# parseablehq/parseable

Hardware: AMD Instinct MI355X
Metric: rows/sec scanned (SELECT...WHERE...GROUP BY, Parseable parquet dialect) (higher is better)
Workload: dtype int64; 1 GPU; c2s; query=SELECT host,count(*),max(latency) WHERE ts BETWEEN ... GROUP BY host, rows_per_gpu=100000000, parallelism=dp1

## Files before the change

### parseable_amd/csrc/gpuq.cpp

```cpp
#include "../../include/gpuq.h"
#include "catalog.h"
#include "where.h"
#include "meta.h"
#include "kernels_api.h"
#include "dev_types.h"

#include <hip/hip_runtime.h>
#include <fcntl.h>
#include <sys/mman.h>
#include <sys/stat.h>
#include <unistd.h>

#include <algorithm>
#include <array>
#include <atomic>
#include <functional>
#include <cstring>
#include <thread>
#include <map>
#include <memory>
#include <mutex>
#include <string>
#include <unordered_map>
#include <vector>
// ... 301 lines not shown
  gpuq_ctx* ctx = nullptr;
  std::vector<std::unique_ptr<MappedFile>> files;
  std::vector<ColPlan> cols;
  std::vector<PredPlan> preds;
  std::vector<AggPlan> aggs;
  std::vector<int> group_cols;
  std::vector<int> projection;
  bool is_projection = false;
  int ts_col = -1;
  int64_t limit = -1;
  std::vector<Partition> parts;
  int32_t n_groups = 0;
  int32_t n_fsum = 0;
  bool has_hash = false;
  bool needs_cascade = false;
  bool has_numkey = false;
  std::vector<std::string> pinned_keys;
  int64_t m_cache_hit_bytes = 0;
  bool fused_count = false;
  bool fused_valagg = false;
  int valagg_col = -1;
  bool valagg_late = false;
  int valagg_blocks = 1024;
  bool exec_dbg = false;
  std::vector<int> distinct_aggs;
  bool has_tree = false;
  WhereTree where;
  std::vector<int> pred_ctx;
  struct WOr { int node; int ctx; int level; std::vector<int> terms; };
  struct WFold { int node; int ctx; int col; };
  struct WCtx { std::vector<int> ors; };
  std::vector<WCtx> ctxs;
  std::vector<WOr> wors;
  std::vector<WFold> wfolds;
  int n_wbufs = 0;
  int ctx_of(int pidx) const { return has_tree ? pred_ctx[pidx] : 0; }
  uint64_t distinct_bitmap_bits = DISTINCT_BITMAP_BITS;
  uint64_t distinct_lds_bits = DISTINCT_LDS_BITS;
  uint32_t distinct_pair_cap = DISTINCT_PAIR_CAP;
  bool distinct_force_hash = false;
  std::mutex mu;
  int64_t m_rows_scanned = 0, m_rows_out = 0, m_kernel_ns = 0, m_exec_ns = 0,
          m_load_ns = 0, m_decomp_ns = 0, m_hbm_est = 0;
  ~gpuq_plan();
};

// ... 1677 lines not shown
            part.dictv_pool[t.dictv_pool_base + k] =
                rank_of_gid[(size_t)part.dictv_pool[t.dictv_pool_base + k]];
  }

  {
    bool aggs_ok = true;
    for (auto& ap : plan->aggs) aggs_ok &= (ap.kind == AGGK_COUNT_STAR);
    plan->fused_count = plan->group_cols.size() == 1 && aggs_ok &&
                        plan->preds.empty() && plan->n_groups <= 8192 &&
                        !plan->cols[plan->group_cols[0]].is_bin &&
                        !plan->cols[plan->group_cols[0]].hash_mode &&
                        !plan->cols[plan->group_cols[0]].numeric_key;
  }

  for (auto& part : plan->parts) {
    part.col_null_free.assign(plan->cols.size(), 1);
    for (auto& t : part.chunks)
      if (t.cm->null_count != 0) part.col_null_free[t.col_idx] = 0;
  }

  plan->exec_dbg = getenv("GPUQ_PLAN_DEBUG") != nullptr;
  if (const char* e = getenv("GPUQ_VALAGG_BLOCKS"))
    plan->valagg_blocks = std::max(1, atoi(e));
  if (const char* e = getenv("GPUQ_DISTINCT_BITMAP_BITS"))
    plan->distinct_bitmap_bits =
        std::min<uint64_t>(strtoull(e, nullptr, 10), 1ull << 31);
  if (const char* e = getenv("GPUQ_DISTINCT_LDS_BITS"))
    plan->distinct_lds_bits =
        std::min<uint64_t>(strtoull(e, nullptr, 10), 64 * 1024 * 8);
  if (const char* e = getenv("GPUQ_DISTINCT_PAIR_CAP"))
    plan->distinct_pair_cap = (uint32_t)std::min<uint64_t>(
        std::max<uint64_t>(strtoull(e, nullptr, 10), 1), DISTINCT_PAIR_CAP);
  if (const char* e = getenv("GPUQ_DISTINCT_FORCE_HASH"))
    plan->distinct_force_hash = atoi(e) != 0;
  if (!plan->distinct_aggs.empty()) plan->fused_count = false;
  if (!plan->is_projection && !getenv("GPUQ_NO_FUSED_VALAGG") &&
      plan->distinct_aggs.empty() &&
      plan->group_cols.size() == 1 && plan->aggs.size() == 2 &&
      plan->aggs[0].kind == AGGK_COUNT_STAR && plan->n_fsum == 0 &&
      (plan->aggs[1].kind == AGGK_SUM_I64 || plan->aggs[1].kind == AGGK_MIN_I64 ||
       plan->aggs[1].kind == AGGK_MAX_I64) &&
      plan->aggs[1].cnt_is_presence && !plan->needs_cascade) {
    const int vc = plan->aggs[1].col_idx;
    const auto& c = plan->cols[vc];
    const auto& kc = plan->cols[plan->group_cols[0]];
    bool ok = c.phys == PT_INT64 && !c.is_bin && !c.hash_mode &&
// ... 800 lines not shown

  {
    std::lock_guard<std::mutex> g(plan->mu);
    plan->m_kernel_ns += (int64_t)(ms_total * 1e6);
    plan->m_decomp_ns += (int64_t)(ms_decomp * 1e6);
    plan->m_exec_ns += now_ns() - t0;
    plan->m_rows_out += k;
  }
  return 0;
}

}

extern "C" int32_t gpuq_plan_execute(gpuq_plan* plan, int32_t pi,
                                     struct ArrowArrayStream* out) try {
  if (!plan || pi < 0 || pi >= (int32_t)plan->parts.size()) return -1;
  Partition& part = plan->parts[pi];
  if (!part.loaded) {
    if (gpuq_plan_load(plan, pi) != 0) return -1;
  }
  HIP_TRY(hipSetDevice(part.device));
  hipStream_t st = part.stream;
  int64_t t0 = now_ns();

  hipEvent_t ev0, ev1, ev_decomp;
  HIP_TRY(hipEventCreate(&ev0));
  HIP_TRY(hipEventCreate(&ev1));
  HIP_TRY(hipEventCreate(&ev_decomp));

  const bool need_mask = !plan->preds.empty() && !part.pred_ranges.empty();
  HIP_TRY(hipMemsetAsync(part.d_err, 0, 4, st));
  if (need_mask) HIP_TRY(hipMemsetAsync(part.d_mask, 1, part.n_rows, st));
  int64_t n_groups_exec = plan->n_groups;
  bool cascaded = false;
  std::vector<uint32_t> level_claimed;
  std::vector<char> distinct_bitmap(plan->distinct_aggs.size(), 0);
  auto key_card = [&](int ci) -> int64_t {
    const auto& kc = plan->cols[ci];
    return kc.is_bin ? (int64_t)kc.nbins + 1
           : (kc.hash_mode || kc.numeric_key)
               ? (int64_t)part.hash_claimed[ci] + 1
               : (int64_t)kc.gdict.size() + 1;
  };
  if (plan->fused_count)
    launch_init_table(st, part.d_table, plan->n_groups, (int)plan->aggs.size(),
                      part.d_agg_kind);
// ... 7 lines not shown
      part.d_res_lane, (int64_t)part.res_lane.size(),
      part.d_res_wave, (int)part.res_wave.size(),
      part.d_piece_pool, part.d_brs,
      part.d_pagebrs, (int)part.pagebrs.size(), part.d_err});
  HIP_TRY(hipEventRecord(ev_decomp, st));

  if (plan->fused_count) {
    int key_col = plan->group_cols[0];
    auto it = part.tasks.find({TK_DICT_GID, key_col});
    if (it != part.tasks.end())
      launch_dict_count(st, part.d_dec, part.d_pages, part.d_ids[it->first],
                        (int)it->second.size(), part.d_remap, part.d_table,
                        plan->n_groups, (int)plan->aggs.size(), part.d_err);
    HIP_TRY(hipEventRecord(ev1, st));
  } else {
  auto run_task = [&](const std::pair<const std::pair<int, int>,
                                      std::vector<int32_t>>& kv,
                      uint8_t* mk) {
    const int kind = tk_kind(kv.first.first), kctx = tk_ctx_of(kv.first.first);
    const int col = kv.first.second;
    int n = (int)kv.second.size();
    int32_t* ids = part.d_ids[kv.first];
    const uint8_t* d_lut = part.d_lut;
    if (kind == TK_DICT_MASK) {
      const auto& lc = plan->cols[col].lut_ctxs;
      d_lut += (size_t)(std::find(lc.begin(), lc.end(), kctx) - lc.begin()) *
               part.lut_pool.size();
    }
    if (part.col_null_free[col]) {
      switch (kind) {
        case TK_DICT_GID: {
          auto it = part.d_valid.find(col);
          launch_dict_gid(st, part.d_dec, part.d_pages, ids, n, part.d_remap,
                          part.d_gid[col],
                          it != part.d_valid.end() ? it->second : nullptr,
                          nullptr, 2, part.d_err);
          return;
        }
        case TK_DICT_VAL:
          launch_dict_i64(st, part.d_dec, part.d_pages, ids, n, part.d_dictv,
                          part.d_val[col], part.d_valid[col], nullptr, 2,
                          part.d_err);
          return;
        case TK_PLAIN_VAL:
          launch_plain_fixed(st, part.d_dec, part.d_pages, ids, n,
                             part.d_val[col], part.d_valid[col], nullptr, 2,
                             part.d_err);
          return;
        case TK_POOL_VAL:
          launch_pool_vals(st, part.d_dec, part.d_pages, ids, n, part.d_dictv,
                           part.d_val[col], part.d_valid[col], nullptr, 2);
          return;
        case TK_DICT_MASK:
          launch_dict_mask(st, part.d_dec, part.d_pages, ids, n, d_lut,
                           mk, 2, part.d_err);
          return;
        default: break;
      }
    }
    switch (kind) {
      case TK_DICT_GID: {
        auto it = part.d_valid.find(col);
        uint8_t* v = it != part.d_valid.end() ? it->second : part.d_tmpvalid;
        launch_def_levels(st, part.d_dec, part.d_pages, ids, n, v, nullptr,
                          nullptr, part.d_rank, part.d_present, part.d_err);
        launch_dict_gid(st, part.d_dec, part.d_pages, ids, n, part.d_remap,
                        part.d_gid[col],
                        it != part.d_valid.end() ? it->second : nullptr,
                        part.d_present, 0, part.d_err);
        launch_dict_gid(st, part.d_dec, part.d_pages, ids, n, part.d_remap,
                        (int32_t*)part.d_scr, nullptr, part.d_present, 1,
                        part.d_err);
        launch_expand(st, part.d_dec, part.d_pages, ids, n, part.d_scr,
                      part.d_rank, v, (uint8_t*)part.d_gid[col], 1);
        break;
      }
      case TK_DICT_VAL:
        launch_def_levels(st, part.d_dec, part.d_pages, ids, n,
                          part.d_valid[col], nullptr, nullptr,
                          part.d_rank, part.d_present, part.d_err);
        launch_dict_i64(st, part.d_dec, part.d_pages, ids, n, part.d_dictv,
                        part.d_val[col], part.d_valid[col], part.d_present, 0,
                        part.d_err);
        launch_dict_i64(st, part.d_dec, part.d_pages, ids, n, part.d_dictv,
                        (int64_t*)part.d_scr, nullptr, part.d_present, 1,
                        part.d_err);
        launch_expand(st, part.d_dec, part.d_pages, ids, n, part.d_scr,
                      part.d_rank, part.d_valid[col],
                      (uint8_t*)part.d_val[col], 0);
        break;
      case TK_PLAIN_VAL:
        launch_def_levels(st, part.d_dec, part.d_pages, ids, n,
                          part.d_valid[col], nullptr, nullptr,
                          part.d_rank, part.d_present, part.d_err);
        launch_plain_fixed(st, part.d_dec, part.d_pages, ids, n,
                           part.d_val[col], part.d_valid[col], part.d_present,
                           0, part.d_err);
        launch_plain_fixed(st, part.d_dec, part.d_pages, ids, n,
                           (int64_t*)part.d_scr, nullptr, part.d_present, 1,
                           part.d_err);
        launch_expand(st, part.d_dec, part.d_pages, ids, n, part.d_scr,
                      part.d_rank, part.d_valid[col],
                      (uint8_t*)part.d_val[col], 0);
        break;
      case TK_POOL_VAL:
        launch_def_levels(st, part.d_dec, part.d_pages, ids, n,
                          part.d_valid[col], nullptr, nullptr,
                          part.d_rank, part.d_present, part.d_err);
        launch_pool_vals(st, part.d_dec, part.d_pages, ids, n, part.d_dictv,
                         part.d_val[col], part.d_valid[col], part.d_present, 0);
        launch_pool_vals(st, part.d_dec, part.d_pages, ids, n, part.d_dictv,
                         (int64_t*)part.d_scr, nullptr, part.d_present, 1);
        launch_expand(st, part.d_dec, part.d_pages, ids, n, part.d_scr,
                      part.d_rank, part.d_valid[col],
                      (uint8_t*)part.d_val[col], 0);
        break;
      case TK_DELTA_VAL:
        launch_delta_i64(st, part.d_dec, part.d_pages, ids, n,
                         part.d_val[col], part.d_valid[col], part.d_err);
        break;
      case TK_DICT_MASK:
        launch_def_levels(st, part.d_dec, part.d_pages, ids, n,
                          part.d_tmpvalid, nullptr, nullptr,
                          part.d_rank, part.d_present, part.d_err);
        launch_dict_mask(st, part.d_dec, part.d_pages, ids, n, d_lut,
                         mk, 0, part.d_err);
        launch_dict_lut_scr(st, part.d_dec, part.d_pages, ids, n, d_lut,
                            part.d_scr, part.d_present, part.d_err);
        launch_expand(st, part.d_dec, part.d_pages, ids, n, part.d_scr,
                      part.d_rank, part.d_tmpvalid, mk, 2);
        break;
      case TK_BYTES_CONTAINS: {
        launch_def_levels(st, part.d_dec, part.d_pages, ids, n,
                          part.d_tmpvalid, mk, part.d_rowof,
                          part.d_rank, part.d_present, part.d_err);
        auto rng = part.cwin_ranges.at(col);
        for (int pidx : plan->cols[col].contains_preds) {
          if (plan->ctx_of(pidx) != kctx) continue;
          const std::string& lit = plan->preds[pidx].str_lit;
          launch_str_win(st, part.d_dec, part.d_cwins + rng.first,
                         (int)rng.second, part.d_pages, part.d_cstarts,
                         part.d_needle + part.needle_off[pidx],
                         (int)lit.size(), like_mode(plan->preds[pidx].p.op),
                         part.d_rowof, mk);
        }
        break;
      }
      case TK_IS_NOT_NULL:
        launch_def_levels(st, part.d_dec, part.d_pages, ids, n,
                          part.d_tmpvalid, mk, nullptr, nullptr,
                          part.d_present, part.d_err);
// ... 215 lines not shown
    a.fsum_idx[i] = ap.fsum_idx;
    if (ap.col_idx >= 0) {
      auto itv = part.d_val.find(ap.col_idx);
      a.agg_val[i] = itv != part.d_val.end() ? itv->second : nullptr;
      auto itd = part.d_valid.find(ap.col_idx);
      a.agg_valid[i] = (ap.cnt_is_presence || itd == part.d_valid.end())
                           ? nullptr : itd->second;
    }
  }
  a.mask = need_mask ? part.d_mask : nullptr;
  a.fsum_n = plan->n_fsum;
  a.fsum = part.d_fsum;
  a.err = part.d_err;
  a.dec = part.d_dec;
  a.table = part.d_table;
  a.n_groups = (int32_t)n_groups_exec;
  launch_init_table(st, part.d_table, (int32_t)n_groups_exec,
                    (int)plan->aggs.size(), part.d_agg_kind);
  if (plan->n_fsum)
    HIP_TRY(hipMemsetAsync(part.d_fsum, 0,
                           (size_t)plan->n_fsum * n_groups_exec * 4 * 8, st));
  bool fused = plan->fused_valagg && n_groups_exec * 16 <= 64 * 1024;
  if (plan->fused_valagg && plan->exec_dbg)
    fprintf(stderr, "[gpuq exec] part %d: valagg=%s n_groups=%lld\n", pi,
            fused ? "fused" : "fallback", (long long)n_groups_exec);
  if (fused) {
    launch_val_agg(st, part.d_dec, part.d_pages, part.d_valagg_ids,
                   (int)part.valagg_ids.size(), part.d_dictv, a.key_gid[0],
                   a.mask, part.d_table, (int32_t)n_groups_exec, a.n_aggs,
                   plan->aggs[1].kind, plan->valagg_blocks, part.d_err);
  } else {
    if (plan->fused_valagg)
      for (auto& kv : part.tasks)
        if (kv.first.second == plan->valagg_col) run_task(kv, part.d_mask);
    launch_agg(st, a);
  }
  for (size_t di = 0; di < plan->distinct_aggs.size(); di++) {
    const int ci = plan->aggs[plan->distinct_aggs[di]].col_idx;
    DistinctArgs d{};
    d.mask = a.mask;
    d.n_rows = part.n_rows;
    d.n_keys = a.n_keys;
    for (int k = 0; k < a.n_keys; k++) {
      d.key_gid[k] = a.key_gid[k];
      d.key_size[k] = a.key_size[k];
    }
    d.n_groups = (int32_t)n_groups_exec;
    d.vgid = part.d_gid[ci];
    d.vcard = (int32_t)key_card(ci);
    d.pairs = part.d_dpairs[di];
    d.count = part.d_dcount + di;
    d.pair_cap = plan->distinct_pair_cap;
    d.err = part.d_err;
// ... 906 lines not shown
```

### parseable_amd/csrc/kernels.hip

```cpp
#include <hip/hip_runtime.h>
#include <cstring>
#include <rocprim/device/device_radix_sort.hpp>
#include "dev_types.h"
#include "meta.h"

namespace gpuq {

#define WAVE 64

#define LZ4_RING 16384
#define LZ4_IN 4096

#define SEG_MAX 8192
__global__ void __launch_bounds__(WAVE)
k_lz4_seg(const uint8_t* __restrict__ raw, uint8_t* __restrict__ dec,
          const DevSeg* __restrict__ segs, int n, int32_t* __restrict__ d_error) {
  __shared__ uint8_t seg[SEG_MAX];
  __shared__ uint8_t inbuf[LZ4_IN + 256];
  int si = blockIdx.x;
  if (si >= n) return;
  const DevSeg sg = segs[si];
  const uint8_t* src = raw + sg.src_off;
  uint8_t* dst = dec + sg.dst_off;
  const int lane = threadIdx.x;
// ... 504 lines not shown
    uint32_t base = tile_base[w >> 3];
    for (uint32_t ww = w & ~7u; ww < w; ww++)
      base += (uint32_t)__popcll(bits[ww]);
    uint32_t r = w * 64 + lane;
    if (r >= nv) break;
    uint8_t ok = (uint8_t)((b >> lane) & 1);
    valid[row0 + r] = ok;
    if (null_mask && !ok) null_mask[row0 + r] = 0;
    uint32_t rk = base + (uint32_t)__popcll(b & lmask);
    if (rankout) rankout[row0 + r] = rk;
    if (rowof && ok) rowof[row0 + rk] = row0 + r;
  }
}

struct EmitGid {
  const int32_t* remap;
  int32_t* out;
  uint8_t* valid;
  __device__ void operator()(uint32_t row, uint32_t idx) const {
    out[row] = remap[idx];
    if (valid) valid[row] = 1;
  }
  __device__ void null_at(uint32_t row) const { out[row] = 0; if (valid) valid[row] = 0; }
};
struct EmitDictI64 {
  const int64_t* dictv;
  int64_t* out;
  uint8_t* valid;
  __device__ void operator()(uint32_t row, uint32_t idx) const { out[row] = dictv[idx]; if (valid) valid[row] = 1; }
  __device__ void null_at(uint32_t row) const { if (valid) valid[row] = 0; }
};
struct EmitDictMask {
  const uint8_t* lut;
  uint8_t* mask;
  __device__ void operator()(uint32_t row, uint32_t idx) const { mask[row] &= lut[idx]; }
  __device__ void null_at(uint32_t row) const { mask[row] = 0; }
};

#define DP_WAVES 4
template <class Emit> struct EmitBatch { static constexpr int N = 1; };
template <class Emit>
__device__ void dict_page_decode(const DevPage& pg, const uint8_t* payload, Emit emit,
                                 const uint32_t* __restrict__ present,
                                 int32_t page_id, int mode, int32_t* d_error) {
  const int lane = threadIdx.x & (WAVE - 1);
  const int wave = threadIdx.x / WAVE;
  const uint8_t* def_start; uint32_t def_len; bool all_valid;
  const uint8_t* vals = def_levels(pg, payload, &def_start, &def_len, &all_valid);
  uint32_t nv = pg.num_values;
  const uint32_t row0 = pg.row_start;
  if (mode == 0) {
    if (!all_valid) return;
  } else if (mode == 1) {
    if (all_valid) return;
    nv = present[page_id];
  }

  {
    int bw = *vals++;
    auto target = [&](uint32_t k) { return row0 + k; };
    if (bw == 0) {
      for (uint32_t i = threadIdx.x; i < nv; i += WAVE * DP_WAVES)
        emit(target(i), 0);
      return;
    }
    const uint8_t* p = vals;
    const uint32_t dict_n = pg.dict_n;
    uint32_t v = 0;
    uint32_t rc = 0;
    while (v < nv) {
      uint64_t hdr = 0; int sh = 0;
      for (;;) {
        uint8_t b = *p++;
        hdr |= (uint64_t)(b & 0x7f) << sh;
        if (!(b & 0x80)) break;
        sh += 7;
      }
      if (hdr & 1) {
        uint32_t groups = (uint32_t)(hdr >> 1);
        uint32_t run_vals = groups * 8;
        if (run_vals > nv - v) run_vals = nv - v;
        const uint32_t mask_v = (bw >= 32) ? 0xffffffffu : ((1u << bw) - 1);
        auto unpack = [&](uint32_t i) -> uint32_t {
          uint32_t g = i >> 3;
          int k = (int)(i & 7);
          const uint8_t* q = p + (size_t)g * bw;
          uint32_t idx;
          if (k * bw + bw <= 64) {
            uint64_t acc;
            __builtin_memcpy(&acc, q, 8);
            idx = (uint32_t)(acc >> (k * bw)) & mask_v;
          } else {
            uint64_t acc2;
            __builtin_memcpy(&acc2, q + (k * bw) / 8, 8);
            idx = (uint32_t)(acc2 >> ((k * bw) % 8)) & mask_v;
          }
          return idx;
        };
        if ((rc++ % DP_WAVES) == (uint32_t)wave) {
          if constexpr (EmitBatch<Emit>::N > 1) {
            constexpr int NB = EmitBatch<Emit>::N;
            for (uint32_t i0 = lane; i0 < run_vals; i0 += WAVE * NB) {
              uint32_t ic[NB], idx[NB];
              uint64_t acc[NB];
#pragma unroll
              for (int u = 0; u < NB; u++) {
                uint32_t i = i0 + u * WAVE;
                ic[u] = i < run_vals ? i : run_vals - 1;
                __builtin_memcpy(&acc[u], p + (((size_t)ic[u] * bw) >> 3), 8);
              }
              bool bad = false;
#pragma unroll
              for (int u = 0; u < NB; u++) {
                idx[u] = (uint32_t)(acc[u] >> ((ic[u] * (uint32_t)bw) & 7)) & mask_v;
                if (idx[u] >= dict_n) { bad = true; idx[u] = 0; }
              }
              if (bad) atomicExch(d_error, ERR_DICT_RANGE);
              typename Emit::Pending pend[NB];
#pragma unroll
              for (int u = 0; u < NB; u++)
                pend[u] = emit.fetch(target(v + ic[u]), idx[u],
                                     i0 + u * WAVE < run_vals);
#pragma unroll
              for (int u = 0; u < NB; u++) emit.apply(pend[u]);
            }
          } else {
            for (uint32_t i = lane; i < run_vals; i += WAVE) {
              uint32_t idx = unpack(i);
              if (idx >= dict_n) { atomicExch(d_error, ERR_DICT_RANGE); idx = 0; }
              emit(target(v + i), idx);
            }
          }
        }
        p += (size_t)groups * bw;
        uint32_t add = groups * 8;
        v += (add > nv - v) ? (nv - v) : add;
      } else {
        uint32_t cnt = (uint32_t)(hdr >> 1);
        uint32_t val = 0;
        int byte_w = (bw + 7) / 8;
        for (int b = 0; b < byte_w; b++) val |= (uint32_t)p[b] << (8 * b);
        p += byte_w;
        if (cnt > nv - v) cnt = nv - v;
        if (val >= dict_n) { if (threadIdx.x == 0) atomicExch(d_error, ERR_DICT_RANGE); val = 0; }
        if ((rc++ % DP_WAVES) == (uint32_t)wave)
        for (uint32_t i = lane; i < cnt; i += WAVE) emit(target(v + i), val);
        v += cnt;
      }
    }
  }
}

template <class Emit>
__global__ void __launch_bounds__(WAVE * DP_WAVES)
k_dict_pages(const uint8_t* __restrict__ dec, const DevPage* __restrict__ pages,
             const int32_t* __restrict__ ids, int n, Emit emit,
             const uint32_t* present, int mode, int32_t* d_error) {
  int pi = blockIdx.x;
  if (pi >= n) return;
  DevPage pg = pages[ids[pi]];
  Emit e = emit;
  e.advance(pg);
  dict_page_decode(pg, dec + pg.dst_off, e, present, ids[pi], mode, d_error);
}

struct EmitGidP : EmitGid {
  const int32_t* pool;
  __device__ void advance(const DevPage& pg) { remap = pool + pg.aux; }
};
struct EmitDictI64P : EmitDictI64 {
  const int64_t* pool;
  __device__ void advance(const DevPage& pg) { dictv = pool + pg.aux_val; }
};
struct EmitDictMaskP : EmitDictMask {
  const uint8_t* pool;
  __device__ void advance(const DevPage& pg) { lut = pool + pg.aux_lut; }
};
struct EmitLutD {
  const uint8_t* pool;
  const uint8_t* lut;
  uint8_t* scr;
  __device__ void operator()(uint32_t row, uint32_t idx) const { scr[row] = lut[idx]; }
  __device__ void null_at(uint32_t) const {}
  __device__ void advance(const DevPage& pg) { lut = pool + pg.aux_lut; }
};

#define FUSED_MAX_GROUPS 8192
__global__ void __launch_bounds__(WAVE)
k_dict_count(const uint8_t* __restrict__ dec, const DevPage* __restrict__ pages,
             const int32_t* __restrict__ ids, int n,
             const int32_t* __restrict__ remap_pool,
             uint64_t* __restrict__ table, int32_t n_groups, int n_aggs,
// ... 1535 lines not shown
    Pending p;
    p.g = gid[row];
    p.v = dictv[idx];
    p.m = MASK ? mask[row] : (uint8_t)1;
    p.on = live;
    return p;
  }
  __device__ void apply(const Pending& p) const {
    if (p.on && p.m) valagg_update<K1>(lt, p.g, p.v);
  }
};
#define VALAGG_BATCH 4
template <int K1, bool MASK> struct EmitBatch<EmitValAgg<K1, MASK>> {
  static constexpr int N = VALAGG_BATCH;
};

template <int K1, bool MASK>
__global__ void __launch_bounds__(WAVE * DP_WAVES)
k_val_agg(const uint8_t* __restrict__ dec, const DevPage* __restrict__ pages,
          const int32_t* __restrict__ ids, int n,
          const int64_t* __restrict__ dictv_pool,
          const int32_t* __restrict__ gid, const uint8_t* __restrict__ mask,
          uint64_t* __restrict__ table, int32_t n_groups, int slots,
          int32_t* d_error) {
  extern __shared__ uint64_t lt[];
  const uint64_t vinit = K1 == AGGK_MIN_I64 ? (uint64_t)INT64_MAX
                         : K1 == AGGK_MAX_I64 ? (uint64_t)INT64_MIN : 0ull;
  for (int i = threadIdx.x; i < 2 * n_groups; i += blockDim.x)
    lt[i] = (i & 1) ? vinit : 0ull;
  __syncthreads();

  for (int pi = blockIdx.x; pi < n; pi += gridDim.x) {
    const DevPage pg = pages[ids[pi]];
    const uint8_t* payload = dec + pg.dst_off;
    if (pg.encoding == ENC_PLAIN) {
      uint32_t skip = 0;
      if (pg.optional) { memcpy(&skip, payload, 4); skip += 4; }
      const uint32_t nv = pg.num_values, row0 = pg.row_start;
      if ((uint64_t)skip + (uint64_t)nv * 8 > pg.uncomp_size) {
        if (threadIdx.x == 0) atomicExch(d_error, ERR_PAGE);
        continue;
      }
      const uint8_t* vals = payload + skip;
      for (uint32_t i0 = threadIdx.x; i0 < nv; i0 += blockDim.x * VALAGG_BATCH) {
        int64_t v[VALAGG_BATCH];
        int32_t g[VALAGG_BATCH];
        uint8_t m[VALAGG_BATCH];
        bool on[VALAGG_BATCH];
#pragma unroll
        for (int u = 0; u < VALAGG_BATCH; u++) {
          uint32_t i = i0 + u * blockDim.x;
          on[u] = i < nv;
          uint32_t row = row0 + (on[u] ? i : i0);
          __builtin_memcpy(&v[u], vals + (size_t)(on[u] ? i : i0) * 8, 8);
          g[u] = gid[row];
          m[u] = MASK ? mask[row] : (uint8_t)1;
        }
#pragma unroll
        for (int u = 0; u < VALAGG_BATCH; u++)
          if (on[u] && m[u]) valagg_update<K1>(lt, g[u], v[u]);
      }
    } else {
      EmitValAgg<K1, MASK> e{dictv_pool + pg.aux_val, gid, mask, lt};
      dict_page_decode(pg, payload, e, (const uint32_t*)nullptr, ids[pi], 2,
                       d_error);
    }
  }
  __syncthreads();
  for (int g = threadIdx.x; g < n_groups; g += blockDim.x) {
    uint64_t c = lt[2 * g];
    if (!c) continue;
    uint64_t* row = table + (int64_t)g * slots;
    atomicAdd((unsigned long long*)&row[0], (unsigned long long)c);
    uint64_t v = lt[2 * g + 1];
    if (K1 == AGGK_SUM_I64) atomicAdd((unsigned long long*)&row[3], (unsigned long long)v);
    else if (K1 == AGGK_MIN_I64) atomic_min_i64(&row[3], (int64_t)v);
    else atomic_max_i64(&row[3], (int64_t)v);
  }
}

__global__ void k_init_table(uint64_t* table, int32_t n_groups, int n_aggs,
                             const int32_t* agg_kind) {
  int slots = 1 + 2 * n_aggs;
  int64_t tsz = (int64_t)n_groups * slots;
  int64_t i = (int64_t)blockIdx.x * blockDim.x + threadIdx.x;
  int64_t stride = (int64_t)gridDim.x * blockDim.x;
  for (; i < tsz; i += stride) {
    int s = (int)(i % slots);
// ... 100 lines not shown
    case STR_SUFFIX: launch(k_affix_win<true>, (int)neg); break;
    default:
      if (fold && neg) launch(k_contains_win<true, true>);
      else if (fold) launch(k_contains_win<true, false>);
      else if (neg) launch(k_contains_win<false, true>);
      else launch(k_contains_win<false, false>);
      break;
  }
}
void launch_null_clear_valid(hipStream_t st, const uint8_t* dec,
                             const DevPage* pages, const int32_t* ids, int n,
                             const uint8_t* valid, uint8_t* mask) {
  if (n) hipLaunchKernelGGL(k_null_clear_valid, dim3(n), dim3(CTHREADS), 0, st, dec, pages, ids, n, valid, mask);
}
void launch_def_levels(hipStream_t st, const uint8_t* dec, const DevPage* pages,
                       const int32_t* ids, int n, uint8_t* valid,
                       uint8_t* null_mask, uint32_t* rowof, uint32_t* rank,
                       uint32_t* present, int32_t* d_err) {
  if (n) hipLaunchKernelGGL(k_def_levels, dim3(n), dim3(WAVE), 0, st, dec, pages, ids, n, valid, null_mask, rowof, rank, present, d_err);
}
void launch_dict_gid(hipStream_t st, const uint8_t* dec, const DevPage* pages,
                     const int32_t* ids, int n, const int32_t* remap_pool,
                     int32_t* out, uint8_t* valid, const uint32_t* present,
                     int mode, int32_t* d_err) {
  if (!n) return;
  EmitGidP e{}; e.pool = remap_pool; e.out = out; e.valid = valid;
  hipLaunchKernelGGL(k_dict_pages<EmitGidP>, dim3(n), dim3(WAVE * DP_WAVES), 0, st, dec, pages, ids, n, e, present, mode, d_err);
}
void launch_dict_i64(hipStream_t st, const uint8_t* dec, const DevPage* pages,
                     const int32_t* ids, int n, const int64_t* dictv_pool,
                     int64_t* out, uint8_t* valid, const uint32_t* present,
                     int mode, int32_t* d_err) {
  if (!n) return;
  EmitDictI64P e{}; e.pool = dictv_pool; e.out = out; e.valid = valid;
  hipLaunchKernelGGL(k_dict_pages<EmitDictI64P>, dim3(n), dim3(WAVE * DP_WAVES), 0, st, dec, pages, ids, n, e, present, mode, d_err);
}
void launch_dict_mask(hipStream_t st, const uint8_t* dec, const DevPage* pages,
                      const int32_t* ids, int n, const uint8_t* lut_pool,
                      uint8_t* mask, int mode, int32_t* d_err) {
  if (!n) return;
  EmitDictMaskP e{}; e.pool = lut_pool; e.mask = mask;
  hipLaunchKernelGGL(k_dict_pages<EmitDictMaskP>, dim3(n), dim3(WAVE * DP_WAVES), 0, st, dec, pages, ids, n, e, (const uint32_t*)nullptr, mode, d_err);
}
void launch_dict_lut_scr(hipStream_t st, const uint8_t* dec,
                         const DevPage* pages, const int32_t* ids, int n,
                         const uint8_t* lut_pool, uint8_t* scr,
                         const uint32_t* present, int32_t* d_err) {
  if (!n) return;
  EmitLutD e{}; e.pool = lut_pool; e.scr = scr;
  hipLaunchKernelGGL(k_dict_pages<EmitLutD>, dim3(n), dim3(WAVE * DP_WAVES), 0, st, dec, pages, ids, n, e, present, 1, d_err);
}
void launch_plain_fixed(hipStream_t st, const uint8_t* dec, const DevPage* pages,
                        const int32_t* ids, int n, int64_t* out, uint8_t* valid,
                        const uint32_t* present, int mode, int32_t* d_err) {
  if (n) hipLaunchKernelGGL(k_plain_fixed, dim3(n), dim3(WAVE), 0, st, dec, pages, ids, n, out, valid, present, mode, d_err);
}
void launch_expand(hipStream_t st, const uint8_t* dec, const DevPage* pages,
                   const int32_t* ids, int n, const uint8_t* scr,
                   const uint32_t* rank, const uint8_t* valid, uint8_t* out,
                   int mode) {
  if (n) hipLaunchKernelGGL(k_expand, dim3(n), dim3(WAVE), 0, st, dec, pages, ids, n, scr, rank, valid, out, mode);
}
void launch_delta_i64(hipStream_t st, const uint8_t* dec, const DevPage* pages,
                      const int32_t* ids, int n, int64_t* out, uint8_t* valid,
                      int32_t* d_err) {
  if (n) hipLaunchKernelGGL(k_delta_i64, dim3(n), dim3(DELTA_T), 0, st, dec, pages, ids, n, out, valid, d_err);
}
void launch_cmp_i64(hipStream_t st, const int64_t* col, const uint8_t* valid,
                    int64_t lo, int64_t hi, int mode, int hi_excl, int is_f64,
                    uint8_t* mask, int64_t n) {
  int blocks = (int)((n + 255) / 256);
  if (blocks > 4096) blocks = 4096;
  if (n) hipLaunchKernelGGL(k_cmp_i64, dim3(blocks), dim3(256), 0, st, col, valid, lo, hi, mode, hi_excl, is_f64, mask, n);
// ... 46 lines not shown

void launch_init_table(hipStream_t st, uint64_t* table, int32_t n_groups,
                       int n_aggs, const int32_t* d_agg_kind) {
  int64_t tsz = (int64_t)n_groups * (1 + 2 * n_aggs);
  int blocks = (int)((tsz + 255) / 256);
  if (blocks > 4096) blocks = 4096;
  hipLaunchKernelGGL(k_init_table, dim3(blocks), dim3(256), 0, st, table, n_groups, n_aggs, d_agg_kind);
}
void launch_dict_count(hipStream_t st, const uint8_t* dec, const DevPage* pages,
                       const int32_t* ids, int n, const int32_t* remap_pool,
                       uint64_t* table, int32_t n_groups, int n_aggs,
                       int32_t* d_err) {
  if (!n) return;
  int blocks = n < 16384 ? n : 16384;
  size_t lds = (size_t)n_groups * 8;
  hipLaunchKernelGGL(k_dict_count, dim3(blocks), dim3(WAVE), lds, st,
                     dec, pages, ids, n, remap_pool, table, n_groups, n_aggs, d_err);
}

void launch_val_agg(hipStream_t st, const uint8_t* dec, const DevPage* pages,
                    const int32_t* ids, int n, const int64_t* dictv_pool,
                    const int32_t* gid, const uint8_t* mask, uint64_t* table,
                    int32_t n_groups, int n_aggs, int kind, int max_blocks,
                    int32_t* d_err) {
  if (!n) return;
  if (max_blocks < 1) max_blocks = 1;
  int per = (n + max_blocks - 1) / max_blocks;
  int blocks = (n + per - 1) / per;
  size_t lds = (size_t)n_groups * 16;
  int slots = 1 + 2 * n_aggs;
  auto launch = [&](auto kern) {
    hipLaunchKernelGGL(kern, dim3(blocks), dim3(WAVE * DP_WAVES), lds, st, dec,
                       pages, ids, n, dictv_pool, gid, mask, table, n_groups,
                       slots, d_err);
  };
  if (mask) {
    switch (kind) {
      case AGGK_SUM_I64: launch(k_val_agg<AGGK_SUM_I64, true>); break;
      case AGGK_MIN_I64: launch(k_val_agg<AGGK_MIN_I64, true>); break;
      default: launch(k_val_agg<AGGK_MAX_I64, true>); break;
    }
  } else {
    switch (kind) {
      case AGGK_SUM_I64: launch(k_val_agg<AGGK_SUM_I64, false>); break;
      case AGGK_MIN_I64: launch(k_val_agg<AGGK_MIN_I64, false>); break;
      default: launch(k_val_agg<AGGK_MAX_I64, false>); break;
    }
  }
}

void launch_agg(hipStream_t st, const AggArgs& a) {
  size_t lds = ((size_t)a.n_groups * (1 + 2 * a.n_aggs) +
                (size_t)a.fsum_n * a.n_groups * 4) * 8;
  int blocks = (int)((a.n_rows + 255) / 256);
  if (blocks > 2048) blocks = 2048;
  if (blocks < 1) blocks = 1;
  bool fast = a.n_keys == 1 && a.n_aggs >= 1 && a.n_aggs <= 2 &&
// ... 172 lines not shown
```

### parseable_amd/csrc/kernels_api.h

```cpp
#pragma once
#include <hip/hip_runtime.h>
#include "dev_types.h"

namespace gpuq {
void launch_lz4_seg(hipStream_t, const uint8_t* raw, uint8_t* dec,
                    const DevSeg*, int n, int32_t* d_err);
void launch_seq_tile(hipStream_t, const uint8_t* raw, uint8_t* dec,
                     const DevSeq* seqs, const DevSeqTile* tiles, int n);
void launch_lit_wave(hipStream_t, const uint8_t* raw, uint8_t* dec,
                     const DevLit* lits, int n);
void launch_lz4_backrefs(hipStream_t, uint8_t* dec, const DevBr*,
                         const DevPageBr*, int n);
void launch_brres_lane(hipStream_t, uint8_t* dec, const DevBrRes*,
                       const DevPiece*, int64_t n);
void launch_brres_wave(hipStream_t, uint8_t* dec, const DevBrRes*,
                       const DevPiece*, int n);
void launch_def_levels(hipStream_t, const uint8_t* dec, const DevPage*,
                       const int32_t* ids, int n, uint8_t* valid,
                       uint8_t* null_mask, uint32_t* rowof, uint32_t* rank,
                       uint32_t* present, int32_t* d_err);
void launch_str_win(hipStream_t, const uint8_t* dec, const DevCWin* wins,
                    int n, const DevPage* pages, const uint16_t* starts_pool,
                    const uint8_t* needle, int nlen, int mode,
                    const uint32_t* rowof, uint8_t* mask);
void launch_null_clear_valid(hipStream_t, const uint8_t* dec, const DevPage*,
                             const int32_t* ids, int n, const uint8_t* valid,
                             uint8_t* mask);
void launch_dict_gid(hipStream_t, const uint8_t* dec, const DevPage*,
                     const int32_t* ids, int n, const int32_t* remap_pool,
                     int32_t* out, uint8_t* valid, const uint32_t* present,
                     int mode, int32_t* d_err);
void launch_dict_i64(hipStream_t, const uint8_t* dec, const DevPage*,
                     const int32_t* ids, int n, const int64_t* dictv_pool,
                     int64_t* out, uint8_t* valid, const uint32_t* present,
                     int mode, int32_t* d_err);
void launch_dict_mask(hipStream_t, const uint8_t* dec, const DevPage*,
                      const int32_t* ids, int n, const uint8_t* lut_pool,
                      uint8_t* mask, int mode, int32_t* d_err);
void launch_dict_lut_scr(hipStream_t, const uint8_t* dec, const DevPage*,
                         const int32_t* ids, int n, const uint8_t* lut_pool,
                         uint8_t* scr, const uint32_t* present, int32_t* d_err);
void launch_plain_fixed(hipStream_t, const uint8_t* dec, const DevPage*,
                        const int32_t* ids, int n, int64_t* out, uint8_t* valid,
                        const uint32_t* present, int mode, int32_t* d_err);
void launch_expand(hipStream_t, const uint8_t* dec, const DevPage*,
                   const int32_t* ids, int n, const uint8_t* scr,
                   const uint32_t* rank, const uint8_t* valid, uint8_t* out,
                   int mode);
void launch_delta_i64(hipStream_t, const uint8_t* dec, const DevPage*,
                      const int32_t* ids, int n, int64_t* out, uint8_t* valid,
                      int32_t* d_err);
void launch_cmp_i64(hipStream_t, const int64_t* col, const uint8_t* valid,
                    int64_t lo, int64_t hi, int mode, int hi_excl, int is_f64,
                    uint8_t* mask, int64_t n);
void launch_mask_or_reset(hipStream_t, uint8_t* acc, uint8_t* tmp, int64_t n);
void launch_mask_and(hipStream_t, uint8_t* dst, const uint8_t* acc, int64_t n);
void launch_bin_i64(hipStream_t, const int64_t* col, const uint8_t* valid,
                    int64_t origin, int64_t stride, int64_t min_idx,
                    int32_t nbins, int32_t* out, int64_t n);
void launch_init_table(hipStream_t, uint64_t* table, int32_t n_groups,
                       int n_aggs, const int32_t* d_agg_kind);
void launch_dict_count(hipStream_t, const uint8_t* dec, const DevPage*,
                       const int32_t* ids, int n, const int32_t* remap_pool,
                       uint64_t* table, int32_t n_groups, int n_aggs,
                       int32_t* d_err);
void launch_val_agg(hipStream_t, const uint8_t* dec, const DevPage*,
                    const int32_t* ids, int n, const int64_t* dictv_pool,
                    const int32_t* gid, const uint8_t* mask, uint64_t* table,
                    int32_t n_groups, int n_aggs, int kind, int max_blocks,
                    int32_t* d_err);
void launch_agg(hipStream_t, const AggArgs&);
void launch_pool_vals(hipStream_t, const uint8_t* dec, const DevPage*,
                      const int32_t* ids, int n, const int64_t* pool,
                      int64_t* out, uint8_t* valid, const uint32_t* present,
                      int mode);
void launch_hash_build(hipStream_t, const uint8_t* dec, const int64_t* refs,
                       const uint8_t* valid, int64_t n_rows, uint64_t* hkeys,
                       int32_t* hgids, int clog2, uint32_t* counter,
                       uint64_t* gid2ref, int32_t gid_cap, int32_t* d_err);
void launch_hash_lookup(hipStream_t, const uint8_t* dec, const int64_t* refs,
                        const uint8_t* valid, int64_t n_rows,
                        const uint64_t* hkeys, const int32_t* hgids, int clog2,
                        int32_t* out_gid);
void launch_pair_build(hipStream_t, const int32_t* a, const int32_t* b,
                       int64_t n_rows, uint64_t* hkeys, int32_t* hgids,
                       int clog2, uint32_t* counter, uint64_t* gid2pair,
                       int32_t gid_cap, int32_t* d_err);
void launch_pair_lookup(hipStream_t, const int32_t* a, const int32_t* b,
                        int64_t n_rows, const uint64_t* hkeys,
                        const int32_t* hgids, int clog2, int32_t* out);
void launch_numhash_build(hipStream_t, const int64_t* vals,
                          const uint8_t* valid, int64_t n_rows,
                          uint64_t* hkeys, int32_t* hgids, int clog2,
// ... 31 lines not shown
```

Baseline: 30.48 billion rows/s.

## Parallelize RLE/bit-packed run header walk in dict page decode via wave ballot

Dictionary page decoding used to walk RLE/bit-packed hybrid headers one at a time, serially. It now uses a wave-wide scan: each lane probes the header byte at a fixed stride and a ballot finds how many consecutive bit-packed runs share the same header, so those runs can be spread across waves in bulk. This targets the serial header-parsing bottleneck on pages made of many short packed runs. It also adds batched fetch/apply for group-id emission (GID_BATCH 4) and an env switch to fall back to the serial walk, at the cost of more complex control flow and extra header probes on pages that don't fit the pattern.

Result: faster. 32.52 billion rows/s, median of 6 (+6.7%).

```diff
diff --git a/parseable_amd/csrc/gpuq.cpp b/parseable_amd/csrc/gpuq.cpp
--- a/parseable_amd/csrc/gpuq.cpp
+++ b/parseable_amd/csrc/gpuq.cpp
@@ -347,6 +347,7 @@
   int valagg_col = -1;
   bool valagg_late = false;
   int valagg_blocks = 1024;
+  bool dict_serial = false;
   bool exec_dbg = false;
   std::vector<int> distinct_aggs;
   bool has_tree = false;
@@ -2070,6 +2071,8 @@
   plan->exec_dbg = getenv("GPUQ_PLAN_DEBUG") != nullptr;
   if (const char* e = getenv("GPUQ_VALAGG_BLOCKS"))
     plan->valagg_blocks = std::max(1, atoi(e));
+  if (const char* e = getenv("GPUQ_DICT_WALK"))
+    plan->dict_serial = strcmp(e, "serial") == 0;
   if (const char* e = getenv("GPUQ_DISTINCT_BITMAP_BITS"))
     plan->distinct_bitmap_bits =
         std::min<uint64_t>(strtoull(e, nullptr, 10), 1ull << 31);
@@ -2916,6 +2919,7 @@
   HIP_TRY(hipSetDevice(part.device));
   hipStream_t st = part.stream;
   int64_t t0 = now_ns();
+  const bool dw = plan->dict_serial;
 
   hipEvent_t ev0, ev1, ev_decomp;
   HIP_TRY(hipEventCreate(&ev0));
@@ -2969,6 +2973,12 @@
     int n = (int)kv.second.size();
     int32_t* ids = part.d_ids[kv.first];
     const uint8_t* d_lut = part.d_lut;
+    if (plan->exec_dbg &&
+        (kind == TK_DICT_GID || kind == TK_DICT_VAL || kind == TK_DICT_MASK))
+      fprintf(stderr,
+              "[gpuq exec] part %d: dict decode col=%s pages=%d dict_walk=%s\n",
+              pi, plan->cols[col].name.c_str(), n,
+              dw ? "serial" : "scan");
     if (kind == TK_DICT_MASK) {
       const auto& lc = plan->cols[col].lut_ctxs;
       d_lut += (size_t)(std::find(lc.begin(), lc.end(), kctx) - lc.begin()) *
@@ -2981,13 +2991,13 @@
           launch_dict_gid(st, part.d_dec, part.d_pages, ids, n, part.d_remap,
                           part.d_gid[col],
                           it != part.d_valid.end() ? it->second : nullptr,
-                          nullptr, 2, part.d_err);
+                          nullptr, 2, dw, part.d_err);
           return;
         }
         case TK_DICT_VAL:
           launch_dict_i64(st, part.d_dec, part.d_pages, ids, n, part.d_dictv,
                           part.d_val[col], part.d_valid[col], nullptr, 2,
-                          part.d_err);
+                          dw, part.d_err);
           return;
         case TK_PLAIN_VAL:
           launch_plain_fixed(st, part.d_dec, part.d_pages, ids, n,
@@ -3000,7 +3010,7 @@
           return;
         case TK_DICT_MASK:
           launch_dict_mask(st, part.d_dec, part.d_pages, ids, n, d_lut,
-                           mk, 2, part.d_err);
+                           mk, 2, dw, part.d_err);
           return;
         default: break;
       }
@@ -3014,10 +3024,10 @@
         launch_dict_gid(st, part.d_dec, part.d_pages, ids, n, part.d_remap,
                         part.d_gid[col],
                         it != part.d_valid.end() ? it->second : nullptr,
-                        part.d_present, 0, part.d_err);
+                        part.d_present, 0, dw, part.d_err);
         launch_dict_gid(st, part.d_dec, part.d_pages, ids, n, part.d_remap,
                         (int32_t*)part.d_scr, nullptr, part.d_present, 1,
-                        part.d_err);
+                        dw, part.d_err);
         launch_expand(st, part.d_dec, part.d_pages, ids, n, part.d_scr,
                       part.d_rank, v, (uint8_t*)part.d_gid[col], 1);
         break;
@@ -3028,10 +3038,10 @@
                           part.d_rank, part.d_present, part.d_err);
         launch_dict_i64(st, part.d_dec, part.d_pages, ids, n, part.d_dictv,
                         part.d_val[col], part.d_valid[col], part.d_present, 0,
-                        part.d_err);
+                        dw, part.d_err);
         launch_dict_i64(st, part.d_dec, part.d_pages, ids, n, part.d_dictv,
                         (int64_t*)part.d_scr, nullptr, part.d_present, 1,
-                        part.d_err);
+                        dw, part.d_err);
         launch_expand(st, part.d_dec, part.d_pages, ids, n, part.d_scr,
                       part.d_rank, part.d_valid[col],
                       (uint8_t*)part.d_val[col], 0);
@@ -3071,9 +3081,9 @@
                           part.d_tmpvalid, nullptr, nullptr,
                           part.d_rank, part.d_present, part.d_err);
         launch_dict_mask(st, part.d_dec, part.d_pages, ids, n, d_lut,
-                         mk, 0, part.d_err);
+                         mk, 0, dw, part.d_err);
         launch_dict_lut_scr(st, part.d_dec, part.d_pages, ids, n, d_lut,
-                            part.d_scr, part.d_present, part.d_err);
+                            part.d_scr, part.d_present, dw, part.d_err);
         launch_expand(st, part.d_dec, part.d_pages, ids, n, part.d_scr,
                       part.d_rank, part.d_tmpvalid, mk, 2);
         break;
@@ -3335,13 +3345,15 @@
                            (size_t)plan->n_fsum * n_groups_exec * 4 * 8, st));
   bool fused = plan->fused_valagg && n_groups_exec * 16 <= 64 * 1024;
   if (plan->fused_valagg && plan->exec_dbg)
-    fprintf(stderr, "[gpuq exec] part %d: valagg=%s n_groups=%lld\n", pi,
-            fused ? "fused" : "fallback", (long long)n_groups_exec);
+    fprintf(stderr,
+            "[gpuq exec] part %d: valagg=%s n_groups=%lld dict_walk=%s\n", pi,
+            fused ? "fused" : "fallback", (long long)n_groups_exec,
+            dw ? "serial" : "scan");
   if (fused) {
     launch_val_agg(st, part.d_dec, part.d_pages, part.d_valagg_ids,
                    (int)part.valagg_ids.size(), part.d_dictv, a.key_gid[0],
                    a.mask, part.d_table, (int32_t)n_groups_exec, a.n_aggs,
-                   plan->aggs[1].kind, plan->valagg_blocks, part.d_err);
+                   plan->aggs[1].kind, plan->valagg_blocks, dw, part.d_err);
   } else {
     if (plan->fused_valagg)
       for (auto& kv : part.tasks)
diff --git a/parseable_amd/csrc/kernels.hip b/parseable_amd/csrc/kernels.hip
--- a/parseable_amd/csrc/kernels.hip
+++ b/parseable_amd/csrc/kernels.hip
@@ -550,6 +550,13 @@
     if (valid) valid[row] = 1;
   }
   __device__ void null_at(uint32_t row) const { out[row] = 0; if (valid) valid[row] = 0; }
+  struct Pending { uint32_t row; int32_t g; bool on; };
+  __device__ Pending fetch(uint32_t row, uint32_t idx, bool live) const {
+    return Pending{row, remap[idx], live};
+  }
+  __device__ void apply(const Pending& p) const {
+    if (p.on) { out[p.row] = p.g; if (valid) valid[p.row] = 1; }
+  }
 };
 struct EmitDictI64 {
   const int64_t* dictv;
@@ -570,7 +577,8 @@
 template <class Emit>
 __device__ void dict_page_decode(const DevPage& pg, const uint8_t* payload, Emit emit,
                                  const uint32_t* __restrict__ present,
-                                 int32_t page_id, int mode, int32_t* d_error) {
+                                 int32_t page_id, int mode, int32_t* d_error,
+                                 bool serial) {
   const int lane = threadIdx.x & (WAVE - 1);
   const int wave = threadIdx.x / WAVE;
   const uint8_t* def_start; uint32_t def_len; bool all_valid;
@@ -593,26 +601,43 @@
       return;
     }
     const uint8_t* p = vals;
+    const uint8_t* const page_end = payload + pg.uncomp_size;
     const uint32_t dict_n = pg.dict_n;
+    const uint32_t mask_v = (bw >= 32) ? 0xffffffffu : ((1u << bw) - 1);
     uint32_t v = 0;
     uint32_t rc = 0;
-    while (v < nv) {
-      uint64_t hdr = 0; int sh = 0;
-      for (;;) {
-        uint8_t b = *p++;
-        hdr |= (uint64_t)(b & 0x7f) << sh;
-        if (!(b & 0x80)) break;
-        sh += 7;
-      }
-      if (hdr & 1) {
-        uint32_t groups = (uint32_t)(hdr >> 1);
-        uint32_t run_vals = groups * 8;
-        if (run_vals > nv - v) run_vals = nv - v;
-        const uint32_t mask_v = (bw >= 32) ? 0xffffffffu : ((1u << bw) - 1);
-        auto unpack = [&](uint32_t i) -> uint32_t {
+    auto packed_run = [&](const uint8_t* q0, uint32_t v0, uint32_t run_vals) {
+      if constexpr (EmitBatch<Emit>::N > 1) {
+        constexpr int NB = EmitBatch<Emit>::N;
+        for (uint32_t i0 = lane; i0 < run_vals; i0 += WAVE * NB) {
+          uint32_t ic[NB], idx[NB];
+          uint64_t acc[NB];
+#pragma unroll
+          for (int u = 0; u < NB; u++) {
+            uint32_t i = i0 + u * WAVE;
+            ic[u] = i < run_vals ? i : run_vals - 1;
+            __builtin_memcpy(&acc[u], q0 + (((size_t)ic[u] * bw) >> 3), 8);
+          }
+          bool bad = false;
+#pragma unroll
+          for (int u = 0; u < NB; u++) {
+            idx[u] = (uint32_t)(acc[u] >> ((ic[u] * (uint32_t)bw) & 7)) & mask_v;
+            if (idx[u] >= dict_n) { bad = true; idx[u] = 0; }
+          }
+          if (bad) atomicExch(d_error, ERR_DICT_RANGE);
+          typename Emit::Pending pend[NB];
+#pragma unroll
+          for (int u = 0; u < NB; u++)
+            pend[u] = emit.fetch(target(v0 + ic[u]), idx[u],
+                                 i0 + u * WAVE < run_vals);
+#pragma unroll
+          for (int u = 0; u < NB; u++) emit.apply(pend[u]);
+        }
+      } else {
+        for (uint32_t i = lane; i < run_vals; i += WAVE) {
           uint32_t g = i >> 3;
           int k = (int)(i & 7);
-          const uint8_t* q = p + (size_t)g * bw;
+          const uint8_t* q = q0 + (size_t)g * bw;
           uint32_t idx;
           if (k * bw + bw <= 64) {
             uint64_t acc;
@@ -623,46 +648,48 @@
             __builtin_memcpy(&acc2, q + (k * bw) / 8, 8);
             idx = (uint32_t)(acc2 >> ((k * bw) % 8)) & mask_v;
           }
-          return idx;
-        };
-        if ((rc++ % DP_WAVES) == (uint32_t)wave) {
-          if constexpr (EmitBatch<Emit>::N > 1) {
-            constexpr int NB = EmitBatch<Emit>::N;
-            for (uint32_t i0 = lane; i0 < run_vals; i0 += WAVE * NB) {
-              uint32_t ic[NB], idx[NB];
-              uint64_t acc[NB];
-#pragma unroll
-              for (int u = 0; u < NB; u++) {
-                uint32_t i = i0 + u * WAVE;
-                ic[u] = i < run_vals ? i : run_vals - 1;
-                __builtin_memcpy(&acc[u], p + (((size_t)ic[u] * bw) >> 3), 8);
-              }
-              bool bad = false;
-#pragma unroll
-              for (int u = 0; u < NB; u++) {
-                idx[u] = (uint32_t)(acc[u] >> ((ic[u] * (uint32_t)bw) & 7)) & mask_v;
-                if (idx[u] >= dict_n) { bad = true; idx[u] = 0; }
-              }
-              if (bad) atomicExch(d_error, ERR_DICT_RANGE);
-              typename Emit::Pending pend[NB];
-#pragma unroll
-              for (int u = 0; u < NB; u++)
-                pend[u] = emit.fetch(target(v + ic[u]), idx[u],
-                                     i0 + u * WAVE < run_vals);
-#pragma unroll
-              for (int u = 0; u < NB; u++) emit.apply(pend[u]);
-            }
-          } else {
-            for (uint32_t i = lane; i < run_vals; i += WAVE) {
-              uint32_t idx = unpack(i);
-              if (idx >= dict_n) { atomicExch(d_error, ERR_DICT_RANGE); idx = 0; }
-              emit(target(v + i), idx);
-            }
+          if (idx >= dict_n) { atomicExch(d_error, ERR_DICT_RANGE); idx = 0; }
+          emit(target(v0 + i), idx);
+        }
+      }
+    };
+    while (v < nv) {
+      uint64_t hdr = 0; int sh = 0;
+      for (;;) {
+        uint8_t b = *p++;
+        hdr |= (uint64_t)(b & 0x7f) << sh;
+        if (!(b & 0x80)) break;
+        sh += 7;
+      }
+      if (hdr & 1) {
+        uint32_t groups = (uint32_t)(hdr >> 1);
+        uint32_t run_vals = groups * 8;
+        if (run_vals > nv - v) run_vals = nv - v;
+        if ((rc++ % DP_WAVES) == (uint32_t)wave) packed_run(p, v, run_vals);
+        p += (size_t)groups * bw;
+        v += run_vals;
+        if (!serial && groups - 1u < 63u) {
+          const uint32_t gv = groups * 8;
+          const uint32_t stride = 1 + groups * (uint32_t)bw;
+          const uint8_t hb = (uint8_t)hdr;
+          for (;;) {
+            const uint32_t full = (nv - v) / gv;
+            const int64_t room = page_end - p;
+            const bool ok = (uint32_t)lane < full &&
+                            (int64_t)(lane + 1) * stride <= room;
+            const uint8_t b = ok ? p[(size_t)lane * stride] : (uint8_t)0;
+            const uint64_t hit = __ballot(ok && b == hb);
+            const uint32_t na =
+                ~hit ? (uint32_t)__builtin_ctzll(~hit) : (uint32_t)WAVE;
+            for (uint32_t j = ((uint32_t)wave + DP_WAVES - rc % DP_WAVES) % DP_WAVES;
+                 j < na; j += DP_WAVES)
+              packed_run(p + (size_t)j * stride + 1, v + j * gv, gv);
+            p += (size_t)na * stride;
+            v += na * gv;
+            rc += na;
+            if (na < (uint32_t)WAVE) break;
           }
         }
-        p += (size_t)groups * bw;
-        uint32_t add = groups * 8;
-        v += (add > nv - v) ? (nv - v) : add;
       } else {
         uint32_t cnt = (uint32_t)(hdr >> 1);
         uint32_t val = 0;
@@ -683,19 +710,22 @@
 __global__ void __launch_bounds__(WAVE * DP_WAVES)
 k_dict_pages(const uint8_t* __restrict__ dec, const DevPage* __restrict__ pages,
              const int32_t* __restrict__ ids, int n, Emit emit,
-             const uint32_t* present, int mode, int32_t* d_error) {
+             const uint32_t* present, int mode, int32_t* d_error, int serial) {
   int pi = blockIdx.x;
   if (pi >= n) return;
   DevPage pg = pages[ids[pi]];
   Emit e = emit;
   e.advance(pg);
-  dict_page_decode(pg, dec + pg.dst_off, e, present, ids[pi], mode, d_error);
+  dict_page_decode(pg, dec + pg.dst_off, e, present, ids[pi], mode, d_error,
+                   serial != 0);
 }
 
 struct EmitGidP : EmitGid {
   const int32_t* pool;
   __device__ void advance(const DevPage& pg) { remap = pool + pg.aux; }
 };
+#define GID_BATCH 4
+template <> struct EmitBatch<EmitGidP> { static constexpr int N = GID_BATCH; };
 struct EmitDictI64P : EmitDictI64 {
   const int64_t* pool;
   __device__ void advance(const DevPage& pg) { dictv = pool + pg.aux_val; }
@@ -2277,7 +2307,7 @@
           const int64_t* __restrict__ dictv_pool,
           const int32_t* __restrict__ gid, const uint8_t* __restrict__ mask,
           uint64_t* __restrict__ table, int32_t n_groups, int slots,
-          int32_t* d_error) {
+          int32_t* d_error, int serial) {
   extern __shared__ uint64_t lt[];
   const uint64_t vinit = K1 == AGGK_MIN_I64 ? (uint64_t)INT64_MAX
                          : K1 == AGGK_MAX_I64 ? (uint64_t)INT64_MIN : 0ull;
@@ -2318,7 +2348,7 @@
     } else {
       EmitValAgg<K1, MASK> e{dictv_pool + pg.aux_val, gid, mask, lt};
       dict_page_decode(pg, payload, e, (const uint32_t*)nullptr, ids[pi], 2,
-                       d_error);
+                       d_error, serial != 0);
     }
   }
   __syncthreads();
@@ -2465,33 +2495,35 @@
 void launch_dict_gid(hipStream_t st, const uint8_t* dec, const DevPage* pages,
                      const int32_t* ids, int n, const int32_t* remap_pool,
                      int32_t* out, uint8_t* valid, const uint32_t* present,
-                     int mode, int32_t* d_err) {
+                     int mode, bool serial_walk, int32_t* d_err) {
   if (!n) return;
   EmitGidP e{}; e.pool = remap_pool; e.out = out; e.valid = valid;
-  hipLaunchKernelGGL(k_dict_pages<EmitGidP>, dim3(n), dim3(WAVE * DP_WAVES), 0, st, dec, pages, ids, n, e, present, mode, d_err);
+  hipLaunchKernelGGL(k_dict_pages<EmitGidP>, dim3(n), dim3(WAVE * DP_WAVES), 0, st, dec, pages, ids, n, e, present, mode, d_err, (int)serial_walk);
 }
 void launch_dict_i64(hipStream_t st, const uint8_t* dec, const DevPage* pages,
                      const int32_t* ids, int n, const int64_t* dictv_pool,
                      int64_t* out, uint8_t* valid, const uint32_t* present,
-                     int mode, int32_t* d_err) {
+                     int mode, bool serial_walk, int32_t* d_err) {
   if (!n) return;
   EmitDictI64P e{}; e.pool = dictv_pool; e.out = out; e.valid = valid;
-  hipLaunchKernelGGL(k_dict_pages<EmitDictI64P>, dim3(n), dim3(WAVE * DP_WAVES), 0, st, dec, pages, ids, n, e, present, mode, d_err);
+  hipLaunchKernelGGL(k_dict_pages<EmitDictI64P>, dim3(n), dim3(WAVE * DP_WAVES), 0, st, dec, pages, ids, n, e, present, mode, d_err, (int)serial_walk);
 }
 void launch_dict_mask(hipStream_t st, const uint8_t* dec, const DevPage* pages,
                       const int32_t* ids, int n, const uint8_t* lut_pool,
-                      uint8_t* mask, int mode, int32_t* d_err) {
+                      uint8_t* mask, int mode, bool serial_walk,
+                      int32_t* d_err) {
   if (!n) return;
   EmitDictMaskP e{}; e.pool = lut_pool; e.mask = mask;
-  hipLaunchKernelGGL(k_dict_pages<EmitDictMaskP>, dim3(n), dim3(WAVE * DP_WAVES), 0, st, dec, pages, ids, n, e, (const uint32_t*)nullptr, mode, d_err);
+  hipLaunchKernelGGL(k_dict_pages<EmitDictMaskP>, dim3(n), dim3(WAVE * DP_WAVES), 0, st, dec, pages, ids, n, e, (const uint32_t*)nullptr, mode, d_err, (int)serial_walk);
 }
 void launch_dict_lut_scr(hipStream_t st, const uint8_t* dec,
                          const DevPage* pages, const int32_t* ids, int n,
                          const uint8_t* lut_pool, uint8_t* scr,
-                         const uint32_t* present, int32_t* d_err) {
+                         const uint32_t* present, bool serial_walk,
+                         int32_t* d_err) {
   if (!n) return;
   EmitLutD e{}; e.pool = lut_pool; e.scr = scr;
-  hipLaunchKernelGGL(k_dict_pages<EmitLutD>, dim3(n), dim3(WAVE * DP_WAVES), 0, st, dec, pages, ids, n, e, present, 1, d_err);
+  hipLaunchKernelGGL(k_dict_pages<EmitLutD>, dim3(n), dim3(WAVE * DP_WAVES), 0, st, dec, pages, ids, n, e, present, 1, d_err, (int)serial_walk);
 }
 void launch_plain_fixed(hipStream_t st, const uint8_t* dec, const DevPage* pages,
                         const int32_t* ids, int n, int64_t* out, uint8_t* valid,
@@ -2584,7 +2616,7 @@
                     const int32_t* ids, int n, const int64_t* dictv_pool,
                     const int32_t* gid, const uint8_t* mask, uint64_t* table,
                     int32_t n_groups, int n_aggs, int kind, int max_blocks,
-                    int32_t* d_err) {
+                    bool serial_walk, int32_t* d_err) {
   if (!n) return;
   if (max_blocks < 1) max_blocks = 1;
   int per = (n + max_blocks - 1) / max_blocks;
@@ -2594,7 +2626,7 @@
   auto launch = [&](auto kern) {
     hipLaunchKernelGGL(kern, dim3(blocks), dim3(WAVE * DP_WAVES), lds, st, dec,
                        pages, ids, n, dictv_pool, gid, mask, table, n_groups,
-                       slots, d_err);
+                       slots, d_err, (int)serial_walk);
   };
   if (mask) {
     switch (kind) {
diff --git a/parseable_amd/csrc/kernels_api.h b/parseable_amd/csrc/kernels_api.h
--- a/parseable_amd/csrc/kernels_api.h
+++ b/parseable_amd/csrc/kernels_api.h
@@ -29,17 +29,18 @@
 void launch_dict_gid(hipStream_t, const uint8_t* dec, const DevPage*,
                      const int32_t* ids, int n, const int32_t* remap_pool,
                      int32_t* out, uint8_t* valid, const uint32_t* present,
-                     int mode, int32_t* d_err);
+                     int mode, bool serial_walk, int32_t* d_err);
 void launch_dict_i64(hipStream_t, const uint8_t* dec, const DevPage*,
                      const int32_t* ids, int n, const int64_t* dictv_pool,
                      int64_t* out, uint8_t* valid, const uint32_t* present,
-                     int mode, int32_t* d_err);
+                     int mode, bool serial_walk, int32_t* d_err);
 void launch_dict_mask(hipStream_t, const uint8_t* dec, const DevPage*,
                       const int32_t* ids, int n, const uint8_t* lut_pool,
-                      uint8_t* mask, int mode, int32_t* d_err);
+                      uint8_t* mask, int mode, bool serial_walk, int32_t* d_err);
 void launch_dict_lut_scr(hipStream_t, const uint8_t* dec, const DevPage*,
                          const int32_t* ids, int n, const uint8_t* lut_pool,
-                         uint8_t* scr, const uint32_t* present, int32_t* d_err);
+                         uint8_t* scr, const uint32_t* present,
+                         bool serial_walk, int32_t* d_err);
 void launch_plain_fixed(hipStream_t, const uint8_t* dec, const DevPage*,
                         const int32_t* ids, int n, int64_t* out, uint8_t* valid,
                         const uint32_t* present, int mode, int32_t* d_err);
@@ -68,7 +69,7 @@
                     const int32_t* ids, int n, const int64_t* dictv_pool,
                     const int32_t* gid, const uint8_t* mask, uint64_t* table,
                     int32_t n_groups, int n_aggs, int kind, int max_blocks,
-                    int32_t* d_err);
+                    bool serial_walk, int32_t* d_err);
 void launch_agg(hipStream_t, const AggArgs&);
 void launch_pool_vals(hipStream_t, const uint8_t* dec, const DevPage*,
                       const int32_t* ids, int n, const int64_t* pool,
```
